# tgale96/sputnik

Hardware: AMD Instinct MI355X
Metric: effective TFLOP/s (nnz-FLOPs) DSD block=128 M=K=N=4096 @ 1/2/4/8 GPU vs density (higher is better)
Workload: dtype f16

## Files before the change

### sputnik_amd/csrc/dsd4w.hip

```cpp
#include <hip/hip_runtime.h>
#include <stdint.h>

#include <cstdlib>

#include "api_internal.h"
#include "block_gemm.h"
#include "dsd4w.h"
#include "dsd4w_asm.inc"

namespace sputnik_amd {
namespace {

constexpr int kRankScratch = 24576;
constexpr uint32_t kOob = 0x80000000u;

struct Pick {
  int row_a, row_b, e_a, n_a, e_b, n_b, target;
  int uniform;
};

__device__ Pick rank_wave(const GemmParams &p, char *lds, int wave, int lane,
                          int ra, int rb, int o0_pre, bool pre) {
  const int R = p.num_rows;
  const int o0 = pre ? o0_pre : lane <= R ? p.s_offsets[lane] : 0;
  const int o1 = __shfl_down(o0, 1, 64);
  const int nr = lane < R ? o1 - o0 : -1;
  int *keys = reinterpret_cast<int *>(lds + kRankScratch + wave * 256);
  int *nbr = reinterpret_cast<int *>(lds + kRankScratch + 2048 + wave * 256);
  const bool live = lane < R;
  const int key = live ? (nr << 6) | (63 - lane) : -1;
  keys[lane] = key;
  int4 k4[16];
#pragma unroll
  for (int j = 0; j < 16; ++j) k4[j] = *reinterpret_cast<const int4 *>(keys + 4 * j);
  int rank = 0;
#pragma unroll
  for (int j = 0; j < 16; ++j)
    rank += (k4[j].x > key) + (k4[j].y > key) + (k4[j].z > key) + (k4[j].w > key);
  const unsigned long long ba = __ballot(live && rank == ra);
  const unsigned long long bb = __ballot(live && rank == rb);
  Pick out;
  out.row_a = __builtin_ctzll(ba);
  out.row_b = __builtin_ctzll(bb);
  out.e_a = __builtin_amdgcn_readlane(o0, out.row_a);
  out.n_a = __builtin_amdgcn_readlane(nr, out.row_a);
  out.e_b = __builtin_amdgcn_readlane(o0, out.row_b);
  out.n_b = __builtin_amdgcn_readlane(nr, out.row_b);
  if (live) nbr[rank] = nr;
  int v = 0;
  if (lane < (R + 1) / 2) {
    const int j = R - 1 - lane;
    v = lane == j ? nbr[lane] : (nbr[lane] + nbr[j] + 1) / 2;
  }
  int vmax = 0;
#pragma unroll
  for (int bit = 15; bit >= 0; --bit) {
    const int cand = vmax | (1 << bit);
    if (__ballot(v >= cand) != 0) vmax = cand;
  }
  out.target = vmax;
  return out;
}

__device__ Pick rank_block(const GemmParams &p, char *lds, int tid, int ra, int rb) {
  const int R = p.num_rows;
  int *offs = reinterpret_cast<int *>(lds + kRankScratch);
  int *n_by_rank = offs + R + 1;
  int *scratch = reinterpret_cast<int *>(lds + kRankScratch + 4096);
  for (int r = tid; r <= R; r += 256) offs[r] = p.s_offsets[r];
  if (tid == 0) {
    scratch[2] = 0;
    scratch[3] = 1;
  }
  __syncthreads();
  const int n0 = offs[1] - offs[0];
  for (int r = tid; r < R; r += 256) {
    const int nr = offs[r + 1] - offs[r];
    if (nr != n0) scratch[3] = 0;
    int rank = 0;
    for (int r2 = 0; r2 < R; ++r2) {
      const int n2 = offs[r2 + 1] - offs[r2];
      rank += (n2 > nr) | ((n2 == nr) & (r2 < r));
    }
    n_by_rank[rank] = nr;
    if (rank == ra) scratch[0] = r;
    if (rank == rb) scratch[1] = r;
  }
  __syncthreads();
  for (int i = tid; i < (R + 1) / 2; i += 256) {
    const int j = R - 1 - i;
    const int v = i == j ? n_by_rank[i] : (n_by_rank[i] + n_by_rank[j] + 1) / 2;
    atomicMax(&scratch[2], v);
  }
  __syncthreads();
  Pick out;
  out.row_a = __builtin_amdgcn_readfirstlane(scratch[0]);
  out.row_b = __builtin_amdgcn_readfirstlane(scratch[1]);
  out.target = __builtin_amdgcn_readfirstlane(scratch[2]);
  out.uniform = __builtin_amdgcn_readfirstlane(scratch[3]);
  out.e_a = __builtin_amdgcn_readfirstlane(offs[out.row_a]);
  out.n_a = __builtin_amdgcn_readfirstlane(offs[out.row_a + 1]) - out.e_a;
  out.e_b = __builtin_amdgcn_readfirstlane(offs[out.row_b]);
  out.n_b = __builtin_amdgcn_readfirstlane(offs[out.row_b + 1]) - out.e_b;
  __syncthreads();
  return out;
}

__device__ __forceinline__ unsigned long long exp_stamp(int dep) {
#if (SPUTNIK_EXP & 512) != 0
  unsigned long long t;
  asm volatile("s_memrealtime %0\n s_waitcnt lgkmcnt(0)"
               : "=s"(t) : "s"(__builtin_amdgcn_readfirstlane(dep)));
  return t;
#else
  (void)dep;
  return 0;
#endif
}

template <bool kBf16, int kEpi, bool kDds, bool kSdd = false, bool kNt = false,
          bool kTt = false, bool kTn = false>
__global__ void __launch_bounds__(256, 1) dsd4w_kernel(const GemmParams p) {
  constexpr bool kWaveEpi = kEpi != 0;
  constexpr bool kDs = kEpi == 3 || kEpi == 4 || kEpi == 5 || kEpi == 6 || kEpi == 7;
  constexpr bool kBar2 = kEpi == 4;
  constexpr bool kKs = kEpi == 6;
  constexpr bool kTp = kEpi == 7;
  static_assert(!kTp || (!kSdd && !kDds && !kNt && !kTt && !kTn), "tall pipeline: DSD NN");
  static_assert(!kDds || kEpi == 1 || kEpi == 3, "DDS: per-wave epilogue only");
  static_assert(!kSdd || ((kEpi == 3 || (kEpi == 4 && !kTt) || (kEpi == 1 && kTn) ||
                           (kKs && !kNt && !kTt && !kTn)) && !kDds),
                "SDD: double slots (TN: per-step images), per-wave epilogue");
  static_assert(!kKs || kSdd, "K-split: SDD NN only");
  constexpr bool kARowsT = (kTt || kTn) && kSdd;
  constexpr bool kDdsTt = kDds && kTt;
  [[maybe_unused]] const unsigned long long t_entry = __builtin_amdgcn_s_memrealtime();
  __shared__ __attribute__((aligned(1024))) char lds[163840];
  const int tid = threadIdx.x;
  const int lane = tid & 63;
  const int wave = __builtin_amdgcn_readfirstlane(tid >> 6);
  const uint32_t lbase =
      (uint32_t)(uintptr_t)((__attribute__((address_space(3))) char *)lds);

  constexpr int kIdxPreload = 1024;
  const int nb_all = p.s_blocks;
  [[maybe_unused]] const unsigned long long t_karg = exp_stamp(nb_all);
  const bool idx_pre = nb_all <= kIdxPreload &&
                       (reinterpret_cast<uintptr_t>(p.s_indices) & 15) == 0;
  typedef unsigned v4u_t __attribute__((ext_vector_type(4)));
  v4u_t idx_lo = {0u, 0u, 0u, 0u}, idx_hi = {0u, 0u, 0u, 0u};
  if (idx_pre) {
    const __amdgpu_buffer_rsrc_t ri = __builtin_amdgcn_make_buffer_rsrc(
        const_cast<short *>(p.s_indices), 0, (nb_all * 2 + 3) & ~3, 0x00020000);
    idx_lo = __builtin_bit_cast(v4u_t, __builtin_amdgcn_raw_buffer_load_b128(
                                            ri, lane * 32, 0, 0));
    idx_hi = __builtin_bit_cast(v4u_t, __builtin_amdgcn_raw_buffer_load_b128(
                                            ri, lane * 32 + 16, 0, 0));
  }
#ifndef SPUTNIK_OFF_EARLY
#define SPUTNIK_OFF_EARLY 1
#endif
  const bool off_early = SPUTNIK_OFF_EARLY && !kSdd && !kTp && p.num_rows < 64;
  int off_pre = 0;
  if (off_early && lane <= p.num_rows) off_pre = p.s_offsets[lane];
  auto kblock_of = [&](int e) {
    if constexpr (kSdd) return e;
    if (!idx_pre || e >= nb_all) return scalar_load_short(p.s_indices, e);
    const int l = e >> 4, d = (e & 15) >> 1;
    const unsigned w0 = __builtin_amdgcn_readlane(idx_lo.x, l);
    const unsigned w1 = __builtin_amdgcn_readlane(idx_lo.y, l);
    const unsigned w2 = __builtin_amdgcn_readlane(idx_lo.z, l);
    const unsigned w3 = __builtin_amdgcn_readlane(idx_lo.w, l);
    const unsigned w4 = __builtin_amdgcn_readlane(idx_hi.x, l);
    const unsigned w5 = __builtin_amdgcn_readlane(idx_hi.y, l);
    const unsigned w6 = __builtin_amdgcn_readlane(idx_hi.z, l);
    const unsigned w7 = __builtin_amdgcn_readlane(idx_hi.w, l);
    const unsigned w = d == 0 ? w0 : d == 1 ? w1 : d == 2 ? w2 : d == 3 ? w3
                     : d == 4 ? w4 : d == 5 ? w5 : d == 6 ? w6 : w7;
    return (int)((e & 1) ? (w >> 16) : (w & 0xffff));
  };

  int srow, j0;
  int b1, n1, b2 = 0, n2 = 0;
  bool producer = false, collect = false;
  int pair_id = 0;
  [[maybe_unused]] unsigned long long t_rank = 0;
  unsigned epoch = p.pair_epoch;
  if (p.pair != 0 && p.pair_sync != nullptr)
    epoch = ((unsigned)scalar_load_int(reinterpret_cast<const int *>(p.pair_sync), 0) &
             0x7fffffffu) + 1u;
  int grp_b0 = 0, grp_count = 0, grp_c = 0;
  bool split_idle = false;
  int kss = 1, kch = 0, kofs = 0;
  unsigned tp_ent = 0, tp_tile = 0, tp_ent2 = 0, tp_tile2 = 0, tp_zero = 0xffffffffu;
  int tp_first = 0, tp_second = 0, tp_nzero = 0;
  if constexpr (kSdd) {
    int tile = xcd_tile(blockIdx.x, gridDim.x);
    const int R = !kKs && p.sdd_tail != 0
                      ? sdd_tail_rows<256>(p, reinterpret_cast<int *>(lds + kRankScratch), tid)
                      : p.num_rows;
    const bool band = p.sdd_order >= 1;
    const int per = band ? ((R + 255) / 256 + 7) & ~7 : (R + 255) / 256;
    const int r0 = min(R, tid * per), r1 = min(R, r0 + per);
    int local = 0, gmin = 0x7fffffff, gmax = 0;
    for (int r = r0; r < r1; ++r) {
      const int gr = (p.c_offsets[r + 1] - p.c_offsets[r] + 3) / 4;
      local += gr;
      gmin = min(gmin, gr);
      gmax = max(gmax, gr);
    }
    int incl = local;
#pragma unroll
    for (int d = 1; d < 64; d <<= 1) {
      const int v = __shfl_up(incl, d, 64);
      if (lane >= d) incl += v;
    }
#pragma unroll
    for (int d = 1; d < 64; d <<= 1) {
      gmin = min(gmin, __shfl_xor(gmin, d, 64));
      gmax = max(gmax, __shfl_xor(gmax, d, 64));
    }
    int *wsum = reinterpret_cast<int *>(lds + kRankScratch);
    if (lane == 63) {
      wsum[wave] = incl;
      wsum[4 + wave] = gmin;
      wsum[8 + wave] = gmax;
    }
    __syncthreads();
    int before = 0, total = 0;
    for (int w2 = 0; w2 < 4; ++w2) {
      const int v = wsum[w2];
      before += w2 < wave ? v : 0;
      total += v;
      gmin = min(gmin, wsum[4 + w2]);
      gmax = max(gmax, wsum[8 + w2]);
    }
    if constexpr (kKs) {
      const int nk = p.k_limit / 128;
      for (int s = 8; s >= 2 && kss == 1; s >>= 1)
        if (s <= p.sdd_ksplit && total * s <= (int)gridDim.x && nk >= 2 * s) kss = s;
      kch = tile / max(total, 1);
      tile -= kch * total;
      if (kch >= kss) tile = total;
    } else {
      tile = (int)blockIdx.x < total ? xcd_tile(blockIdx.x, total) : total;
    }
    int start = before + incl - local;
    const bool uniform = gmin == gmax;
    if (!uniform && band && total >= 8 * R) {
      for (int rb0 = r0; rb0 < r1; rb0 += 8) {
        int g8[8], bt = 0;
#pragma unroll
        for (int i = 0; i < 8; ++i) {
          g8[i] = rb0 + i < r1 ? (p.c_offsets[rb0 + i + 1] - p.c_offsets[rb0 + i] + 3) / 4 : 0;
          bt += g8[i];
        }
        if (tile >= start && tile < start + bt) {
          int o = tile - start, lo = 0;
          for (int it = 0; it < 8; ++it) {
            int cnt = 0, m = 0x7fffffff;
#pragma unroll
            for (int i = 0; i < 8; ++i)
              if (g8[i] > lo) {
                ++cnt;
                m = min(m, g8[i]);
              }
            if (o < cnt * (m - lo)) {
              const int k = o % cnt;
              int row = rb0, c = 0;
#pragma unroll
              for (int i = 0; i < 8; ++i)
                if (g8[i] > lo) {
                  if (c == k) row = rb0 + i;
                  ++c;
                }
              wsum[12] = row;
              wsum[13] = lo + o / cnt;
              break;
            }
            o -= cnt * (m - lo);
            lo = m;
          }
        }
        start += bt;
      }
    } else if (!uniform) {
      for (int r = r0; r < r1; ++r) {
        const int gr = (p.c_offsets[r + 1] - p.c_offsets[r] + 3) / 4;
        if (tile >= start && tile < start + gr) {
          wsum[12] = r;
          wsum[13] = tile - start;
        }
        start += gr;
      }
    }
    __syncthreads();
    j0 = 0;
    b1 = 0;
    n1 = p.k_limit / 128;
    srow = 0;
    if (tile >= total) {
      if (!kKs || p.pair == 0 || p.pair_sync == nullptr) return;
      split_idle = true;
    } else {
      int gi;
      const int gpr = total / max(R, 1);
      const int rb = p.sdd_order == 2 ? 4 : p.sdd_order == 3 ? 16 : p.sdd_order == 4 ? 32 : 8;
      const int gb = 32 / rb;
      if (uniform && p.sdd_order >= 1 && R % rb == 0 && gpr % gb == 0) {
        const int sup = tile >> 5, w = tile & 31;
        const int ngs = gpr / gb;
        srow = (sup / ngs) * rb + (w % rb);
        gi = p.sdd_spread ? (w / rb) * ngs + (sup % ngs) : (sup % ngs) * gb + (w / rb);
      } else if (uniform) {
        srow = tile % R;
        gi = tile / R;
      } else {
        srow = __builtin_amdgcn_readfirstlane(wsum[12]);
        gi = __builtin_amdgcn_readfirstlane(wsum[13]);
      }
      grp_b0 = __builtin_amdgcn_readfirstlane(p.c_offsets[srow] + gi * 4);
      grp_count = __builtin_amdgcn_readfirstlane(min(4, p.c_offsets[srow + 1] - grp_b0));
      grp_c = scalar_load_short(p.c_indices, grp_b0 + min(wave, grp_count - 1));
      if constexpr (kKs) {
        const int c0 = kch * n1 / kss, c1 = (kch + 1) * n1 / kss;
        kofs = c0;
        n1 = c1 - c0;
        pair_id = tile * kss;
      } else if (p.sdd_krot != 0 && n1 > 1) {
        const int key = p.sdd_krot == 1 ? srow : p.sdd_krot == 2 ? gi
                        : p.sdd_krot == 3 ? tile : srow >> 3;
        const int rot = (int)(((unsigned)key * 17u) % (unsigned)n1);
        b1 = rot;
        b2 = 0;
        n2 = rot;
        n1 -= rot;
      }
    }
    __syncthreads();
  } else if constexpr (kTp) {
    const int kFlushW = p.tall_flush_w;
    const int R = p.num_rows, NB = nb_all, P = p.num_jtiles;
    const int G = gridDim.x;
    const int w = xcd_tile(blockIdx.x, G);
    int *loff = reinterpret_cast<int *>(lds);
    int *wsc = reinterpret_cast<int *>(lds + kRankScratch + 131072);
    for (int r = tid; r <= R; r += 256) loff[r] = p.s_offsets[r];
    __syncthreads();
    const int per = (R + 255) / 256;
    const int r0 = min(R, tid * per), r1 = min(R, r0 + per);
    int local = 0;
    for (int r = r0; r < r1; ++r) local += loff[r + 1] == loff[r] ? 1 : 0;
    int incl = local;
#pragma unroll
    for (int d = 1; d < 64; d <<= 1) {
      const int v = __shfl_up(incl, d, 64);
      if (lane >= d) incl += v;
    }
    if (lane == 63) wsc[wave] = incl;
    __syncthreads();
    int before = 0, E = 0;
    for (int w2 = 0; w2 < 4; ++w2) {
      before += w2 < wave ? wsc[w2] : 0;
      E += wsc[w2];
    }
    const int NE = R - E;
    const long long W = 4LL * NB + (long long)kFlushW * NE;
    const long long TW = (long long)P * W;
    const int rot = xcd_rotation();
    auto share = [&](int ww) -> long long {
      long long acc = 0;
      int base = 0;
      for (int x = 0; x < 8; ++x) {
        const int nx = G / 8 + (x < G % 8 ? 1 : 0);
        const long long sx = fast_xcd(x, rot) ? p.tall_odd_share : 100;
        if (ww <= base + nx) return acc + (long long)(ww - base) * sx;
        acc += (long long)nx * sx;
        base += nx;
      }
      return acc;
    };
    const long long stot = share(G), sw0 = share(w), sw1 = share(w + 1);
    const long long lo0 = TW * sw0 / stot, lo1 = TW * sw1 / stot;
    const long long q0 = lo0 / max(W, 1LL), q1 = lo1 / max(W, 1LL);
    const long long rem0 = lo0 - q0 * W, rem1 = lo1 - q1 * W;
    long long m0 = (long long)NB, m1 = (long long)NB, k0 = 0x7fffffffffffLL, k1 = k0;
    {
      int e = before + incl - local;
      for (int r = r0; r < r1; ++r) {
        if (loff[r + 1] == loff[r]) {
          ++e;
          continue;
        }
        const long long key = 4LL * loff[r] + (long long)kFlushW * (r - e);
        if (key >= rem0 && key < k0) { k0 = key; m0 = loff[r]; }
        if (key >= rem1 && key < k1) { k1 = key; m1 = loff[r]; }
      }
    }
#pragma unroll
    for (int d = 1; d < 64; d <<= 1) {
      const long long ok0 = __shfl_xor(k0, d, 64), om0 = __shfl_xor(m0, d, 64);
      const long long ok1 = __shfl_xor(k1, d, 64), om1 = __shfl_xor(m1, d, 64);
      if (ok0 < k0) { k0 = ok0; m0 = om0; }
      if (ok1 < k1) { k1 = ok1; m1 = om1; }
    }
    long long *wk = reinterpret_cast<long long *>(wsc + 8);
    if (lane == 0) {
      wk[4 * wave] = k0;
      wk[4 * wave + 1] = m0;
      wk[4 * wave + 2] = k1;
      wk[4 * wave + 3] = m1;
    }
    __syncthreads();
    for (int w2 = 0; w2 < 4; ++w2) {
      if (wk[4 * w2] < k0) { k0 = wk[4 * w2]; m0 = wk[4 * w2 + 1]; }
      if (wk[4 * w2 + 2] < k1) { k1 = wk[4 * w2 + 2]; m1 = wk[4 * w2 + 3]; }
    }
    const long long T = (long long)P * NB;
    const long long b0 = min(T, q0 * NB + m0);
    const long long b1g = w + 1 == G ? T : min(T, q1 * NB + m1);
    const int nblk = (int)min(128LL, max(0LL, b1g - b0));
    auto describe = [&](int x, unsigned &ent, unsigned &til) {
      ent = 0;
      til = 0;
      if (x >= nblk) return;
      const long long g = b0 + x;
      const int q = (int)(g / NB), e = (int)(g - (long long)q * NB);
      int lo = 0, hi = R;
      while (hi - lo > 1) {
        const int mid = (lo + hi) >> 1;
        if (loff[mid] <= e) lo = mid; else hi = mid;
      }
      const bool last = e == loff[lo + 1] - 1;
      ent = (unsigned)e | ((unsigned)q << 24);
      til = (unsigned)lo | ((unsigned)q << 16) | (last ? 0x80000000u : 0u);
    };
    describe(lane, tp_ent, tp_tile);
    describe(64 + lane, tp_ent2, tp_tile2);
    {
      const long long Z = (long long)P * E;
      const int zlo = (int)(Z * sw0 / stot), zhi = (int)(Z * sw1 / stot);
      int *zl = wsc + 48;
      int e = before + incl - local;
      for (int r = r0; r < r1; ++r) {
        if (loff[r + 1] != loff[r]) continue;
        for (int q = 0; q < P; ++q) {
          const long long rank = (long long)q * E + e;
          if (rank >= zlo && rank < zhi) zl[rank - zlo] = r | (q << 16);
        }
        ++e;
      }
      __syncthreads();
      tp_nzero = min(64, zhi - zlo);
      tp_zero = lane < tp_nzero ? (unsigned)zl[lane] : 0xffffffffu;
    }
    __syncthreads();
    j0 = 0;
    srow = 0;
    b1 = 0;
    n1 = nblk;
    tp_first = (int)(__builtin_amdgcn_readlane(tp_ent, 0) & 0xffffffu);
    tp_second = (int)(__builtin_amdgcn_readlane(tp_ent, nblk > 1 ? 1 : 0) & 0xffffffu);
    split_idle = nblk == 0;
  } else if (p.pair != 0 && p.pair_split == 2) {
    const int nt = p.num_tiles;
    const int gch = (int)blockIdx.x >= nt ? 1 : 0;
    const int t = xcd_tile((int)blockIdx.x - gch * nt, nt);
    srow = t % p.num_rows;
    j0 = (t / p.num_rows) * 512;
    const int e_r = scalar_load_int(p.s_offsets, srow);
    const int n_r = scalar_load_int(p.s_offsets, srow + 1) - e_r;
    const int c0 = gch * n_r / 2, c1 = (gch + 1) * n_r / 2;
    b1 = e_r + c0;
    n1 = c1 - c0;
    pair_id = t;
    if (gch == 0) {
      producer = n1 > 0;
      split_idle = n1 == 0;
    } else {
      collect = n_r / 2 > 0;
    }
  } else if (p.pair != 0) {
    const int R = p.num_rows;
    const int half = R >> 1;
    const int n_light = p.num_jtiles * half;
    const int n_solo = p.num_jtiles * (R & 1);
    const int bid = blockIdx.x;
    int role, panel, pi;
    const bool xcd2 = p.pair_xcd2 != 0 && p.num_jtiles == 8 && n_solo == 0 &&
                      (half & 1) == 0;
    const int rot = xcd2 ? xcd_rotation() : 0;
    auto place = [&](int b) {
      if (xcd2) {
        const int x = b & 7, k = b >> 3;
        panel = 2 * (x >> 1) + (k & 1);
        pi = p.pair_xcd2 == 2 ? 2 * (k >> 1) + (x & 1)
           : (fast_xcd(x, rot) ^ (p.pair_xcd2 == 3 ? 1 : 0)) * (half >> 1) + (k >> 1);
      } else {
        const int t = xcd_tile(b, n_light);
        panel = t / half;
        pi = t % half;
      }
    };
    if (bid < n_light) {
      role = 0;
      place(bid);
    } else if (bid < n_light + n_solo) {
      role = 1;
      panel = bid - n_light;
      pi = half;
    } else {
      role = 2;
      place(bid - n_light - n_solo);
    }
    const Pick rp = R < 64 ? rank_wave(p, lds, wave, lane, pi, R - 1 - pi, off_pre, off_early)
                           : rank_block(p, lds, tid, pi, R - 1 - pi);
    t_rank = exp_stamp(rp.target + rp.e_a + rp.e_b);
    const int min_handoff = p.min_handoff > 0 ? p.min_handoff : SPUTNIK_MIN_HANDOFF;
    int hb = role == 1 ? 0 : rp.n_a - rp.target;
    if (hb < min_handoff) hb = 0;
    pair_id = panel * half + pi;
    j0 = panel * 512;
    if (role == 0) {
      srow = rp.row_b;
      b1 = rp.e_a;
      n1 = hb;
      b2 = rp.e_b;
      n2 = rp.n_b;
      producer = hb > 0;
    } else {
      srow = rp.row_a;
      b1 = rp.e_a + hb;
      n1 = rp.n_a - hb;
      collect = hb > 0;
    }
  } else {
    const int tile = xcd_tile(blockIdx.x, gridDim.x);
    const int panel = tile / p.num_rows;
    const int target = tile % p.num_rows;
    j0 = panel * 512;
    if (p.num_rows < 64) {
      const Pick rp = rank_wave(p, lds, wave, lane, target, target, off_pre, off_early);
      srow = rp.row_a;
      b1 = rp.e_a;
      n1 = rp.n_a;
    } else if (p.num_rows <= kLptRows) {
      const Pick rp = rank_block(p, lds, tid, target, target);
      srow = rp.row_a;
      b1 = rp.e_a;
      n1 = rp.n_a;
      const int R = p.num_rows;
      if (p.xcd_rows != 0 && rp.uniform != 0 && (R & 7) == 0 &&
          (int)gridDim.x == p.num_tiles) {
        const int rx = R >> 3, x = (int)blockIdx.x & 7, tx = (int)blockIdx.x >> 3;
        srow = x * rx + tx % rx;
        j0 = (tx / rx) * 512;
        const int *offs = reinterpret_cast<const int *>(lds + kRankScratch);
        b1 = __builtin_amdgcn_readfirstlane(offs[srow]);
      }
    } else {
      srow = target;
      b1 = scalar_load_int(p.s_offsets, srow);
      n1 = scalar_load_int(p.s_offsets, srow + 1) - b1;
    }
  }
  srow = __builtin_amdgcn_readfirstlane(srow);
  j0 = __builtin_amdgcn_readfirstlane(j0);
  const int ntot = n1 + n2;

  typedef unsigned v4u __attribute__((ext_vector_type(4)));
  if (split_idle) {
  } else if (ntot == 0 && kDds) {
    const v4u z = {0u, 0u, 0u, 0u};
    for (int id = tid; id < 512 * 16; id += 256) {
      const int r = id >> 4, cc = id & 15;
      if (j0 + r >= p.j_limit) continue;
      __builtin_nontemporal_store(
          z, reinterpret_cast<v4u *>(p.c_data + (long long)(j0 + r) * p.c_ld +
                                     (long long)srow * 256 + cc * 16));
    }
  } else if (ntot == 0) {
    const v4u z = {0u, 0u, 0u, 0u};
    for (int id = tid; id < 128 * 64; id += 256) {
      const int r = id >> 6, cc = id & 63;
      const int jc = j0 + cc * 8;
      if (jc >= p.j_limit) continue;
      __builtin_nontemporal_store(
          z, reinterpret_cast<v4u *>(p.c_data + ((long long)srow * 128 + r) * p.c_ld +
                                     (long long)jc * 2));
    }
  } else {
    const int b2m = b2 - n1;
    const int xlast = ntot - 1;
    auto entry = [&](int x) { return x + (x < n1 ? b1 : b2m); };
    const int kb0 = kblock_of(kTp ? tp_first : entry(0));
    const int kb1 = kblock_of(kTp ? tp_second : entry(xlast < 1 ? xlast : 1));
    constexpr bool kColOrder =
        !kDdsTt && ((kDds && !kNt) || ((kTn || kTt) && !kSdd));
    const int bo0 = kColOrder ? scalar_load_int(p.s_block_offsets, entry(0)) : 0;
    const int bo1 =
        kColOrder ? scalar_load_int(p.s_block_offsets, entry(xlast < 1 ? xlast : 1)) : 0;
    [[maybe_unused]] const unsigned long long t_kb = exp_stamp(kb0 + kb1);

    uint32_t vs, vs1 = 0;
    if constexpr (!kDdsTt && ((kDds && !kNt) || kTt || kTn)) {
      const int k = 8 * wave + (lane >> 4);
      const int pc = lane & 15;
      const int c = (((pc >> 1) ^ tr_key(k)) << 1) | (pc & 1);
      vs = (uint32_t)(k * (kARowsT ? p.s_ld : 256) + c * 16);
    } else if constexpr (kDs) {
      const long long srs = kSdd ? p.s_ld : 256;
      auto off = [&](int x) {
        const int r = 32 * wave + 8 * x + (lane >> 3);
        return (uint32_t)(r * srs + (((lane & 7) ^ ((r >> 1) & 7)) << 4));
      };
      vs = off(0);
      vs1 = off(1);
    } else {
      const int srow_l = 32 * wave + (lane >> 2);
      vs = (uint32_t)(srow_l * 256 + (((lane & 3) ^ ((srow_l >> 1) & 3)) << 4));
    }
    uint32_t vd[2];
#pragma unroll
    for (int x = 0; x < 2; ++x) {
      if constexpr (!kDdsTt && ((kDds && kDs) || kNt || kTt)) {
        const int r = 8 * x + (lane >> 3);
        vd[x] = j0 + 128 * wave < p.j_limit
                    ? (uint32_t)(r * p.d_ld + (((lane & 7) ^ ((r >> 1) & 7)) << 4))
                    : kOob;
      } else if constexpr (kDds && !kTn && !kDdsTt) {
        const int r = lane >> 2;
        vd[x] = j0 + 128 * wave < p.j_limit
                    ? (uint32_t)(r * p.d_ld + (((lane & 3) ^ ((r >> 1) & 3)) << 4))
                    : kOob;
      } else {
        const int k = (lane >> 4) + 8 * x;
        const int pc = lane & 15;
        const int c = (((pc >> 1) ^ tr_key(k)) << 1) | (pc & 1);
        const int col = (kSdd ? grp_c * 128 : j0 + 128 * wave) + c * 8;
        vd[x] = col < p.j_limit ? (uint32_t)((lane >> 4) * p.d_ld + c * 16) : kOob;
      }
    }
    const uint32_t own = lbase + 32768u + 32768u * wave;
    const int r16 = lane & 15, g = lane >> 4;
    const uint32_t vrs =
        (kDds ? own : lbase) +
        (kDs ? (uint32_t)(r16 * 128 + ((g ^ ((r16 >> 1) & 7)) << 4))
             : (uint32_t)(r16 * 64 + ((g ^ ((r16 >> 1) & 3)) << 4)));
    const uint32_t vrs1 = vrs ^ 64u;
    const int q = (lane >> 2) & 3, pp = lane & 3;
    const int kr = 8 * g + q;
    uint32_t vrd[8];
#pragma unroll
    for (int n = 0; n < 8; ++n)
      vrd[n] = (kDds || kTt ? lbase : own) +
               (uint32_t)(kr * 256 + pp * 8 + ((n ^ tr_key(kr)) << 5));
    uint32_t vrt[8];
#pragma unroll
    for (int m = 0; m < 8; ++m)
      vrt[m] = (kDds ? own : lbase) +
               (uint32_t)(kr * 256 + pp * 8 + ((m ^ tr_key(kr)) << 5));
    const uint32_t vrk0 = (kDds ? lbase : own) +
                          (uint32_t)(r16 * 128 + ((g ^ ((r16 >> 1) & 7)) << 4));
    const uint32_t vrk1 = vrk0 ^ 64u;
    const uint32_t vw0 = lbase + (uint32_t)(r16 * 1040 + (128 * wave + 4 * g) * 2);
    const uint32_t vw1 = vw0 + 64 * 1040;
    const uint32_t wreg = lbase + 32768u + 32768u * wave;
    uint32_t vws[8], vrb[4];
#pragma unroll
    for (int n = 0; n < 8; ++n)
      vws[n] = wreg + (uint32_t)(r16 * 256 + (((2 * n + (g >> 1)) ^ r16) << 4) + 8 * (g & 1));
#pragma unroll
    for (int qq = 0; qq < 4; ++qq) {
      const int rr = 4 * qq + g;
      vrb[qq] = wreg + (uint32_t)(rr * 256 + ((r16 ^ rr) << 4));
    }
    const bool cvalid = kSdd   ? wave < grp_count
                        : kDds ? j0 + 128 * wave < p.j_limit
                               : j0 + 128 * wave + r16 * 8 < p.j_limit;
    const long long cld = kSdd ? 256 : p.c_ld;
    const uint32_t vco = cvalid ? (uint32_t)(g * cld + r16 * 16) : kOob;
    const uint32_t vpl = (uint32_t)(wave * 65536 + lane * 16);
    const uint32_t vcl = (uint32_t)((lane & 15) * p.c_ld + (lane >> 4) * 8);

    auto U = [](uint32_t x) { return (uint32_t)__builtin_amdgcn_readfirstlane((int)x); };
    auto U64 = [&](uint64_t x) {
      return (uint64_t)U((uint32_t)x) | ((uint64_t)U((uint32_t)(x >> 32)) << 32);
    };
    const uint64_t sd = U64((uint64_t)(
        p.s_data + (kARowsT ? (long long)srow * 256
                    : kSdd  ? (long long)srow * 128 * p.s_ld + (long long)kofs * 256 : 0)));
    const uint64_t dt = U64((uint64_t)(
        p.d_data + (kDdsTt ? (long long)(j0 + 128 * wave) * 2
                    : (kNt || kTt) && !kSdd ? (long long)(j0 + 128 * wave) * p.d_ld
                    : kNt || kTt ? (long long)grp_c * 128 * p.d_ld
                    : kSdd ? (long long)grp_c * 256 + (long long)kofs * 128 * p.d_ld
                           : (long long)(j0 + 128 * wave) * (kDds && !kTn ? p.d_ld : 2))));
    const uint64_t ix = U64((uint64_t)p.s_indices);
    const uint64_t pd =
        U64((uint64_t)(p.pair_partials + (long long)pair_id * 128 * 512));
    const uint64_t flag_p =
        U64(kKs ? (uint64_t)(p.ks_flags + pair_id)
            : p.pair != 0 ? (uint64_t)(p.pair_flags + pair_id) : 0);
    const uint64_t err_p = U64((uint64_t)p.pair_error);
    constexpr bool kKcD = !kDdsTt && ((kDds && !kTn) || kNt || kTt);
    const uint32_t k128 = U((uint32_t)(kKcD ? 256 : 128 * p.d_ld));
    const uint32_t k32 = U((uint32_t)(kKcD ? 64 : 32 * p.d_ld));
    const uint32_t k4 = U((uint32_t)(kKcD ? 16 * p.d_ld : 4 * p.d_ld));
    const uint32_t ms =
        U(lbase + ((kDs && (((!kDds || kNt) && !kTt) || kDdsTt)) ? 4096u : 2048u) * wave);
    const uint32_t sk32 = U((uint32_t)(kARowsT ? 32 * p.s_ld : 0));
    const uint32_t sk128 = U((uint32_t)(kARowsT ? 128 * p.s_ld : 0));
    const uint32_t md = U(lbase + 32768u + 32768u * wave);
    const uint32_t flushrem = U(producer ? (uint32_t)n2 : 0xffffffffu);
    const uint32_t pubat = U(producer && n2 > 0 ? (uint32_t)n2 + 1u : 0u);
    const uint32_t publast = U(producer && n2 == 0 ? 1u : 0u);
    const bool clb = collect && ntot >= 3;
    const uint32_t clbf = U(clb ? 2u : 0xffffffffu), clbc = U(clb ? 1u : 0xffffffffu);
    const bool split_first = p.pair != 0 && p.pair_split == 2 && producer;
    const uint32_t flags =
        U((collect ? 1u : 0u) | (!collect && !(producer && n2 == 0) ? 2u : 0u) |
          (p.pair_fault ? 4u : 0u) | (wave == 3 ? 8u : 0u) | (wave == 0 ? 16u : 0u) |
          (split_first ? 32u : 0u) | (kKs && wave >= grp_count ? 64u : 0u));
    const uint64_t cd = U64(
        kSdd ? (uint64_t)(p.c_data + (long long)(grp_b0 + wave) * 32768)
        : kDds ? (uint64_t)(p.c_data + (long long)(j0 + 128 * wave) * p.c_ld +
                          (long long)srow * 256)
             : (uint64_t)(p.c_data + (long long)srow * 128 * p.c_ld +
                          (long long)(j0 + 128 * wave) * 2));
    const uint64_t bo = U64((uint64_t)p.s_block_offsets);
    const uint32_t c4 = U((uint32_t)(4 * cld));
    const uint32_t s16 = U((uint32_t)(kARowsT ? 4 * p.s_ld : kSdd ? 16 * p.s_ld : 0));
    const uint32_t ub1 = U(b1), un1 = U(n1), ub2m = U(b2m), uxlast = U(xlast),
                   untot = U(ntot), ukb0 = U(kb0), ukb1 = U(kb1), uep = U(epoch),
                   ubo0 = U(bo0), ubo1 = U(bo1), ukss = U(kss), ukch = U(kch);
    const uint32_t crow = U((uint32_t)(128 * p.c_ld));
    const uint32_t unz = U((uint32_t)tp_nzero);

#define DSD4W_INPUTS                                                           \
    [sdlo] "s"((uint32_t)sd), [sdhi] "s"((uint32_t)(sd >> 32)),               \
    [dtlo] "s"((uint32_t)dt), [dthi] "s"((uint32_t)(dt >> 32)),               \
    [k128] "s"(k128), [k32] "s"(k32), [k4] "s"(k4),                            \
    [ixlo] "s"((uint32_t)ix), [ixhi] "s"((uint32_t)(ix >> 32)),               \
    [b1] "s"(ub1), [n1] "s"(un1), [b2m] "s"(ub2m), [xlast] "s"(uxlast),        \
    [ntot] "s"(untot), [kb0] "s"(ukb0), [kb1] "s"(ukb1),                       \
    [flushrem] "s"(flushrem),                                                  \
    [pdlo] "s"((uint32_t)pd), [pdhi] "s"((uint32_t)(pd >> 32)),               \
    [flag] "s"(flag_p), [epoch] "s"(uep), [flags] "s"(flags),                  \
    [err] "s"(err_p), [ms] "s"(ms),                                            \
    [md] "s"(md), [vs] "v"(vs), [vd0] "v"(vd[0]), [vd1] "v"(vd[1]),           \
    [vrs] "v"(vrs), [vrd0] "v"(vrd[0]), [vrd1] "v"(vrd[1]),                   \
    [vs1] "v"(vs1), [vrs1] "v"(vrs1), [s16] "s"(s16),                          \
    [vrk0] "v"(vrk0), [vrk1] "v"(vrk1), [sk32] "s"(sk32), [sk128] "s"(sk128),  \
    [vrt0] "v"(vrt[0]), [vrt1] "v"(vrt[1]), [vrt2] "v"(vrt[2]), [vrt3] "v"(vrt[3]), \
    [vrt4] "v"(vrt[4]), [vrt5] "v"(vrt[5]), [vrt6] "v"(vrt[6]), [vrt7] "v"(vrt[7]), \
    [vrd2] "v"(vrd[2]), [vrd3] "v"(vrd[3]), [vrd4] "v"(vrd[4]),               \
    [vrd5] "v"(vrd[5]), [vrd6] "v"(vrd[6]), [vrd7] "v"(vrd[7]),               \
    [vpl] "v"(vpl), [bolo] "s"((uint32_t)bo), [bohi] "s"((uint32_t)(bo >> 32)),  \
    [bo0] "s"(ubo0), [bo1] "s"(ubo1), [pubat] "s"(pubat), [clbf] "s"(clbf),  \
    [clbc] "s"(clbc), [publast] "s"(publast), [kss] "s"(ukss), [kch] "s"(ukch), \
    [vent] "v"(tp_ent), [vtile] "v"(tp_tile), [vent2] "v"(tp_ent2),         \
    [vtile2] "v"(tp_tile2), [vcl] "v"(vcl), [crow] "s"(crow),                \
    [vzero] "v"(tp_zero), [nzero] "s"(unz)
#define DSD4W_OPERANDS : DSD4W_INPUTS
#define DSD4W_OPERANDS_G DSD4W_OPERANDS, [vw0] "v"(vw0), [vw1] "v"(vw1)
#define DSD4W_INPUTS_W                                                         \
  DSD4W_INPUTS, [cdlo] "s"((uint32_t)cd), [cdhi] "s"((uint32_t)(cd >> 32)),  \
      [c4] "s"(c4), [vws0] "v"(vws[0]), [vws1] "v"(vws[1]), [vws2] "v"(vws[2]), \
      [vws3] "v"(vws[3]), [vws4] "v"(vws[4]), [vws5] "v"(vws[5]),               \
      [vws6] "v"(vws[6]), [vws7] "v"(vws[7]), [vrb0] "v"(vrb[0]),               \
      [vrb1] "v"(vrb[1]), [vrb2] "v"(vrb[2]), [vrb3] "v"(vrb[3]), [vco] "v"(vco)
#define DSD4W_OPERANDS_W : DSD4W_INPUTS_W
#define DSD4W_RECORD(ROLE, EXTRA)                                              \
  if (p.debug != nullptr && wave == 0 && lane < 16) {                          \
    unsigned long long v = 0;                                                  \
    v = lane == 0 ? t_entry : v;                                               \
    v = lane == 1 ? t_asm : v;                                                 \
    v = lane == 2 ? r0 : v;                                                    \
    v = lane == 3 ? r1 : v;                                                    \
    v = lane == 4 ? r2 : v;                                                    \
    v = lane == 5 ? (unsigned long long)ntot : v;                              \
    v = lane == 6 ? (ROLE) : v;                                                \
    v = lane == 7 ? (unsigned long long)srow : v;                              \
    v = lane == 8 ? (unsigned long long)n1 : v;                                \
    v = lane == 9 ? r3 : v;                                                    \
    v = lane == 10 ? r4 : v;                                                   \
    v = lane == 11 ? t_karg : v;                                               \
    v = lane == 12 ? t_rank : v;                                               \
    v = lane == 13 ? t_kb : v;                                                 \
    v = lane == 14 ? (EXTRA) : v;                                              \
    p.debug[blockIdx.x * 16 + lane] = v;                                       \
  }
    if constexpr (kDdsTt) {
      if constexpr (kBf16)
        asm volatile(DSD4W_ASM_BF16_W2_DDS_TT : DSD4W_OPERANDS_W : DSD4W_CLOBBERS);
      else
        asm volatile(DSD4W_ASM_F16_W2_DDS_TT : DSD4W_OPERANDS_W : DSD4W_CLOBBERS);
    } else if constexpr (kTt && !kSdd) {
      if constexpr (kBf16)
        asm volatile(DSD4W_ASM_BF16_W2_TT : DSD4W_OPERANDS_W : DSD4W_CLOBBERS);
      else
        asm volatile(DSD4W_ASM_F16_W2_TT : DSD4W_OPERANDS_W : DSD4W_CLOBBERS);
    } else if constexpr (kTn && kSdd) {
      if constexpr (kBf16)
        asm volatile(DSD4W_ASM_BF16_W_SDD_TN : DSD4W_OPERANDS_W : DSD4W_CLOBBERS);
      else
        asm volatile(DSD4W_ASM_F16_W_SDD_TN : DSD4W_OPERANDS_W : DSD4W_CLOBBERS);
    } else if constexpr (kTn && kDds) {
      if constexpr (kBf16)
        asm volatile(DSD4W_ASM_BF16_W_DDS_TN : DSD4W_OPERANDS_W : DSD4W_CLOBBERS);
      else
        asm volatile(DSD4W_ASM_F16_W_DDS_TN : DSD4W_OPERANDS_W : DSD4W_CLOBBERS);
    } else if constexpr (kTn) {
      if constexpr (kBf16)
        asm volatile(DSD4W_ASM_BF16_W_TN : DSD4W_OPERANDS_W : DSD4W_CLOBBERS);
      else
        asm volatile(DSD4W_ASM_F16_W_TN : DSD4W_OPERANDS_W : DSD4W_CLOBBERS);
    } else if constexpr (kTt) {
      if constexpr (kBf16)
        asm volatile(DSD4W_ASM_BF16_W2_SDD_TT : DSD4W_OPERANDS_W : DSD4W_CLOBBERS);
      else
        asm volatile(DSD4W_ASM_F16_W2_SDD_TT : DSD4W_OPERANDS_W : DSD4W_CLOBBERS);
    } else if constexpr (kNt && kDds) {
      if constexpr (kBf16)
        asm volatile(DSD4W_ASM_BF16_W2_DDS_NT : DSD4W_OPERANDS_W : DSD4W_CLOBBERS);
      else
        asm volatile(DSD4W_ASM_F16_W2_DDS_NT : DSD4W_OPERANDS_W : DSD4W_CLOBBERS);
    } else if constexpr (kNt && !kSdd) {
      if constexpr (kBf16)
        asm volatile(DSD4W_ASM_BF16_W2_NT : DSD4W_OPERANDS_W : DSD4W_CLOBBERS);
      else
        asm volatile(DSD4W_ASM_F16_W2_NT : DSD4W_OPERANDS_W : DSD4W_CLOBBERS);
    } else if constexpr (kNt && kBar2) {
      if constexpr (kBf16)
        asm volatile(DSD4W_ASM_BF16_W3_SDD_NT : DSD4W_OPERANDS_W : DSD4W_CLOBBERS);
      else
        asm volatile(DSD4W_ASM_F16_W3_SDD_NT : DSD4W_OPERANDS_W : DSD4W_CLOBBERS);
    } else if constexpr (kNt) {
      if constexpr (kBf16)
        asm volatile(DSD4W_ASM_BF16_W2_SDD_NT : DSD4W_OPERANDS_W : DSD4W_CLOBBERS);
      else
        asm volatile(DSD4W_ASM_F16_W2_SDD_NT : DSD4W_OPERANDS_W : DSD4W_CLOBBERS);
    } else if constexpr (kTp && (SPUTNIK_EXP & 512) != 0) {
      const unsigned long long t_asm = __builtin_amdgcn_s_memrealtime();
      unsigned long long r0 = 0, r1 = 0, r2 = 0, r3 = 0, r4 = 0;
      if constexpr ((SPUTNIK_EXP & 1024) != 0)
        asm volatile(DSD4W_ASM_F16_W2_TP_NS : [r0] "=&s"(r0), [r1] "=&s"(r1),
                     [r2] "=&s"(r2), [r3] "=&s"(r3), [r4] "=&s"(r4)
                     : DSD4W_INPUTS_W : DSD4W_CLOBBERS);
      else if constexpr (kBf16)
        asm volatile(DSD4W_ASM_BF16_W2_TP_T : [r0] "=&s"(r0), [r1] "=&s"(r1),
                     [r2] "=&s"(r2), [r3] "=&s"(r3), [r4] "=&s"(r4)
                     : DSD4W_INPUTS_W : DSD4W_CLOBBERS);
      else
        asm volatile(DSD4W_ASM_F16_W2_TP_T : [r0] "=&s"(r0), [r1] "=&s"(r1),
                     [r2] "=&s"(r2), [r3] "=&s"(r3), [r4] "=&s"(r4)
                     : DSD4W_INPUTS_W : DSD4W_CLOBBERS);
      const unsigned long long ntl = (unsigned long long)(
          __popcll(__ballot((tp_tile >> 31) != 0)) + __popcll(__ballot((tp_tile2 >> 31) != 0)));
      DSD4W_RECORD((unsigned long long)tp_nzero, ntl);
    } else if constexpr (kTp) {
      if constexpr (kBf16)
        asm volatile(DSD4W_ASM_BF16_W2_TP : DSD4W_OPERANDS_W : DSD4W_CLOBBERS);
      else
        asm volatile(DSD4W_ASM_F16_W2_TP : DSD4W_OPERANDS_W : DSD4W_CLOBBERS);
    } else if constexpr (kKs && (SPUTNIK_EXP & 512) != 0) {
      const unsigned long long t_asm = __builtin_amdgcn_s_memrealtime();
      unsigned long long r0 = 0, r1 = 0, r2 = 0, r3 = 0, r4 = 0;
      if constexpr (kBf16)
        asm volatile(DSD4W_ASM_BF16_W2_SDD_KS_T : [r0] "=&s"(r0), [r1] "=&s"(r1),
                     [r2] "=&s"(r2), [r3] "=&s"(r3), [r4] "=&s"(r4)
                     : DSD4W_INPUTS_W : DSD4W_CLOBBERS);
      else
        asm volatile(DSD4W_ASM_F16_W2_SDD_KS_T : [r0] "=&s"(r0), [r1] "=&s"(r1),
                     [r2] "=&s"(r2), [r3] "=&s"(r3), [r4] "=&s"(r4)
                     : DSD4W_INPUTS_W : DSD4W_CLOBBERS);
      DSD4W_RECORD((unsigned long long)kch, (unsigned long long)kss);
    } else if constexpr (kKs) {
      if constexpr (kBf16)
        asm volatile(DSD4W_ASM_BF16_W2_SDD_KS : DSD4W_OPERANDS_W : DSD4W_CLOBBERS);
      else
        asm volatile(DSD4W_ASM_F16_W2_SDD_KS : DSD4W_OPERANDS_W : DSD4W_CLOBBERS);
    } else if constexpr (kSdd && kBar2) {
      if constexpr (kBf16)
        asm volatile(DSD4W_ASM_BF16_W3_SDD : DSD4W_OPERANDS_W : DSD4W_CLOBBERS);
      else
        asm volatile(DSD4W_ASM_F16_W3_SDD : DSD4W_OPERANDS_W : DSD4W_CLOBBERS);
    } else if constexpr (kSdd) {
      if constexpr (kBf16)
        asm volatile(DSD4W_ASM_BF16_W2_SDD : DSD4W_OPERANDS_W : DSD4W_CLOBBERS);
      else
        asm volatile(DSD4W_ASM_F16_W2_SDD : DSD4W_OPERANDS_W : DSD4W_CLOBBERS);
    } else if constexpr (kDds && kDs && (SPUTNIK_EXP & 512) != 0) {
      const unsigned long long t_asm = __builtin_amdgcn_s_memrealtime();
      unsigned long long r0 = 0, r1 = 0, r2 = 0, r3 = 0, r4 = 0;
      if constexpr (kBf16)
        asm volatile(DSD4W_ASM_BF16_W2_DDS_T : [r0] "=&s"(r0), [r1] "=&s"(r1),
                     [r2] "=&s"(r2), [r3] "=&s"(r3), [r4] "=&s"(r4)
                     : DSD4W_INPUTS_W : DSD4W_CLOBBERS);
      else
        asm volatile(DSD4W_ASM_F16_W2_DDS_T : [r0] "=&s"(r0), [r1] "=&s"(r1),
                     [r2] "=&s"(r2), [r3] "=&s"(r3), [r4] "=&s"(r4)
                     : DSD4W_INPUTS_W : DSD4W_CLOBBERS);
      DSD4W_RECORD((unsigned long long)((collect ? 2 : 0) | (producer ? 1 : 0)), 0ull);
    } else if constexpr (kDds && kDs) {
      if constexpr (kBf16)
        asm volatile(DSD4W_ASM_BF16_W2_DDS : DSD4W_OPERANDS_W : DSD4W_CLOBBERS);
      else
        asm volatile(DSD4W_ASM_F16_W2_DDS : DSD4W_OPERANDS_W : DSD4W_CLOBBERS);
    } else if constexpr (kDds) {
      if constexpr (kBf16)
        asm volatile(DSD4W_ASM_BF16_W_DDS : DSD4W_OPERANDS_W : DSD4W_CLOBBERS);
      else
        asm volatile(DSD4W_ASM_F16_W_DDS : DSD4W_OPERANDS_W : DSD4W_CLOBBERS);
    } else if constexpr ((SPUTNIK_EXP & 512) != 0 &&
                         (kEpi == 1 || kEpi == 3 || kEpi == 5)) {
      const unsigned long long t_asm = __builtin_amdgcn_s_memrealtime();
      unsigned long long r0 = 0, r1 = 0, r2 = 0, r3 = 0, r4 = 0;
#define DSD4W_STAMPED(NAME)                                                    \
  asm volatile(NAME : [r0] "=&s"(r0), [r1] "=&s"(r1), [r2] "=&s"(r2),          \
               [r3] "=&s"(r3), [r4] "=&s"(r4)                                  \
               : DSD4W_INPUTS_W : DSD4W_CLOBBERS)
      if constexpr (kEpi == 5) {
        if constexpr (kBf16) DSD4W_STAMPED(DSD4W_ASM_BF16_W4_T);
        else DSD4W_STAMPED(DSD4W_ASM_F16_W4_T);
      } else if constexpr (kEpi == 3) {
        if constexpr (kBf16) DSD4W_STAMPED(DSD4W_ASM_BF16_W2_T);
        else DSD4W_STAMPED(DSD4W_ASM_F16_W2_T);
      } else {
        if constexpr (kBf16) DSD4W_STAMPED(DSD4W_ASM_BF16_W_T);
        else DSD4W_STAMPED(DSD4W_ASM_F16_W_T);
      }
#undef DSD4W_STAMPED
      DSD4W_RECORD((unsigned long long)((collect ? 2 : 0) | (producer ? 1 : 0)), 0ull);
    } else if constexpr (kEpi == 5) {
      if constexpr (kBf16)
        asm volatile(DSD4W_ASM_BF16_W4 : DSD4W_OPERANDS_W : DSD4W_CLOBBERS);
      else
        asm volatile(DSD4W_ASM_F16_W4 : DSD4W_OPERANDS_W : DSD4W_CLOBBERS);
    } else if constexpr (kBar2) {
      if constexpr (kBf16)
        asm volatile(DSD4W_ASM_BF16_W3 : DSD4W_OPERANDS_W : DSD4W_CLOBBERS);
      else
        asm volatile(DSD4W_ASM_F16_W3 : DSD4W_OPERANDS_W : DSD4W_CLOBBERS);
    } else if constexpr (kDs) {
      if constexpr (kBf16)
        asm volatile(DSD4W_ASM_BF16_W2 : DSD4W_OPERANDS_W : DSD4W_CLOBBERS);
      else
        asm volatile(DSD4W_ASM_F16_W2 : DSD4W_OPERANDS_W : DSD4W_CLOBBERS);
    } else if constexpr (kEpi == 2) {
      if constexpr (kBf16)
        asm volatile(DSD4W_ASM_BF16_WL : DSD4W_OPERANDS_W : DSD4W_CLOBBERS);
      else
        asm volatile(DSD4W_ASM_F16_WL : DSD4W_OPERANDS_W : DSD4W_CLOBBERS);
    } else if constexpr (kWaveEpi) {
      if constexpr (kBf16)
        asm volatile(DSD4W_ASM_BF16_W : DSD4W_OPERANDS_W : DSD4W_CLOBBERS);
      else
        asm volatile(DSD4W_ASM_F16_W : DSD4W_OPERANDS_W : DSD4W_CLOBBERS);
    } else {
      if constexpr (kBf16)
        asm volatile(DSD4W_ASM_BF16 : DSD4W_OPERANDS_G : DSD4W_CLOBBERS);
      else
        asm volatile(DSD4W_ASM_F16 : DSD4W_OPERANDS_G : DSD4W_CLOBBERS);
      __syncthreads();
      for (int id = tid; id < 128 * 64; id += 256) {
        const int r = id >> 6, cc = id & 63;
        const int jc = j0 + cc * 8;
        if (jc >= p.j_limit) continue;
        const v4u v = *reinterpret_cast<const v4u *>(lds + r * 1040 + cc * 16);
        __builtin_nontemporal_store(
            v, reinterpret_cast<v4u *>(p.c_data + ((long long)srow * 128 + r) * p.c_ld +
                                       (long long)jc * 2));
      }
    }
#undef DSD4W_RECORD
#undef DSD4W_OPERANDS_W
#undef DSD4W_INPUTS_W
#undef DSD4W_OPERANDS_G
#undef DSD4W_OPERANDS
#undef DSD4W_INPUTS
  }
  if constexpr (kTp) {
    typedef unsigned v4z __attribute__((ext_vector_type(4)));
    const v4z z = {0u, 0u, 0u, 0u};
    int jz = 0;
    if (!split_idle) {
// ... 205 lines not shown
```

Measured before the change: 1184.

## Hoist per-lane LDS address setup ahead of scheduling and use DPP reductions

New measurement: 1190 (median of 6 runs). Within noise of the previous version (+0.5%).

```diff
diff --git a/sputnik_amd/csrc/dsd4w.hip b/sputnik_amd/csrc/dsd4w.hip
--- a/sputnik_amd/csrc/dsd4w.hip
+++ b/sputnik_amd/csrc/dsd4w.hip
@@ -26,7 +26,6 @@
   const int o1 = __shfl_down(o0, 1, 64);
   const int nr = lane < R ? o1 - o0 : -1;
   int *keys = reinterpret_cast<int *>(lds + kRankScratch + wave * 256);
-  int *nbr = reinterpret_cast<int *>(lds + kRankScratch + 2048 + wave * 256);
   const bool live = lane < R;
   const int key = live ? (nr << 6) | (63 - lane) : -1;
   keys[lane] = key;
@@ -46,19 +45,17 @@
   out.n_a = __builtin_amdgcn_readlane(nr, out.row_a);
   out.e_b = __builtin_amdgcn_readlane(o0, out.row_b);
   out.n_b = __builtin_amdgcn_readlane(nr, out.row_b);
-  if (live) nbr[rank] = nr;
+  const int by_rank = __builtin_amdgcn_ds_permute(rank << 2, live ? nr : 0);
+  const int j = R - 1 - lane;
+  const int partner = __builtin_amdgcn_ds_bpermute(j << 2, by_rank);
   int v = 0;
-  if (lane < (R + 1) / 2) {
-    const int j = R - 1 - lane;
-    v = lane == j ? nbr[lane] : (nbr[lane] + nbr[j] + 1) / 2;
-  }
-  int vmax = 0;
-#pragma unroll
-  for (int bit = 15; bit >= 0; --bit) {
-    const int cand = vmax | (1 << bit);
-    if (__ballot(v >= cand) != 0) vmax = cand;
-  }
-  out.target = vmax;
+  if (lane < (R + 1) / 2) v = lane == j ? by_rank : (by_rank + partner + 1) / 2;
+  v = max(v, __builtin_amdgcn_update_dpp(0, v, 0xB1, 0xf, 0xf, true));
+  v = max(v, __builtin_amdgcn_update_dpp(0, v, 0x4E, 0xf, 0xf, true));
+  v = max(v, __builtin_amdgcn_update_dpp(0, v, 0x141, 0xf, 0xf, true));
+  v = max(v, __builtin_amdgcn_update_dpp(0, v, 0x140, 0xf, 0xf, true));
+  out.target = max(max(__builtin_amdgcn_readlane(v, 0), __builtin_amdgcn_readlane(v, 16)),
+                   max(__builtin_amdgcn_readlane(v, 32), __builtin_amdgcn_readlane(v, 48)));
   return out;
 }
 
@@ -167,18 +164,98 @@
     if constexpr (kSdd) return e;
     if (!idx_pre || e >= nb_all) return scalar_load_short(p.s_indices, e);
     const int l = e >> 4, d = (e & 15) >> 1;
-    const unsigned w0 = __builtin_amdgcn_readlane(idx_lo.x, l);
-    const unsigned w1 = __builtin_amdgcn_readlane(idx_lo.y, l);
-    const unsigned w2 = __builtin_amdgcn_readlane(idx_lo.z, l);
-    const unsigned w3 = __builtin_amdgcn_readlane(idx_lo.w, l);
-    const unsigned w4 = __builtin_amdgcn_readlane(idx_hi.x, l);
-    const unsigned w5 = __builtin_amdgcn_readlane(idx_hi.y, l);
-    const unsigned w6 = __builtin_amdgcn_readlane(idx_hi.z, l);
-    const unsigned w7 = __builtin_amdgcn_readlane(idx_hi.w, l);
-    const unsigned w = d == 0 ? w0 : d == 1 ? w1 : d == 2 ? w2 : d == 3 ? w3
-                     : d == 4 ? w4 : d == 5 ? w5 : d == 6 ? w6 : w7;
+    const v4u_t h = (d & 4) ? idx_hi : idx_lo;
+    const unsigned h0 = (d & 2) ? h.z : h.x, h1 = (d & 2) ? h.w : h.y;
+    const unsigned w = __builtin_amdgcn_readlane((d & 1) ? h1 : h0, l);
     return (int)((e & 1) ? (w >> 16) : (w & 0xffff));
   };
+
+  uint32_t vs, vs1 = 0;
+  if constexpr (!kDdsTt && ((kDds && !kNt) || kTt || kTn)) {
+    const int k = 8 * wave + (lane >> 4);
+    const int pc = lane & 15;
+    const int c = (((pc >> 1) ^ tr_key(k)) << 1) | (pc & 1);
+    vs = (uint32_t)(k * (kARowsT ? p.s_ld : 256) + c * 16);
+  } else if constexpr (kDs) {
+    const long long srs = kSdd ? p.s_ld : 256;
+    auto off = [&](int x) {
+      const int r = 32 * wave + 8 * x + (lane >> 3);
+      return (uint32_t)(r * srs + (((lane & 7) ^ ((r >> 1) & 7)) << 4));
+    };
+    vs = off(0);
+    vs1 = off(1);
+  } else {
+    const int srow_l = 32 * wave + (lane >> 2);
+    vs = (uint32_t)(srow_l * 256 + (((lane & 3) ^ ((srow_l >> 1) & 3)) << 4));
+  }
+  uint32_t vd_off[2], vd_col[2];
+#pragma unroll
+  for (int x = 0; x < 2; ++x) {
+    if constexpr (!kDdsTt && ((kDds && kDs) || kNt || kTt)) {
+      const int r = 8 * x + (lane >> 3);
+      vd_off[x] = (uint32_t)(r * p.d_ld + (((lane & 7) ^ ((r >> 1) & 7)) << 4));
+      vd_col[x] = (uint32_t)(128 * wave);
+    } else if constexpr (kDds && !kTn && !kDdsTt) {
+      const int r = lane >> 2;
+      vd_off[x] = (uint32_t)(r * p.d_ld + (((lane & 3) ^ ((r >> 1) & 3)) << 4));
+      vd_col[x] = (uint32_t)(128 * wave);
+    } else {
+      const int k = (lane >> 4) + 8 * x;
+      const int pc = lane & 15;
+      const int c = (((pc >> 1) ^ tr_key(k)) << 1) | (pc & 1);
+      vd_off[x] = (uint32_t)((lane >> 4) * p.d_ld + c * 16);
+      vd_col[x] = (uint32_t)((kSdd ? 0 : 128 * wave) + c * 8);
+    }
+  }
+  const uint32_t own = lbase + 32768u + 32768u * wave;
+  const int r16 = lane & 15, g = lane >> 4;
+  uint32_t vrs =
+      (kDds ? own : lbase) +
+      (kDs ? (uint32_t)(r16 * 128 + ((g ^ ((r16 >> 1) & 7)) << 4))
+           : (uint32_t)(r16 * 64 + ((g ^ ((r16 >> 1) & 3)) << 4)));
+  uint32_t vrs1 = vrs ^ 64u;
+  const int q = (lane >> 2) & 3, pp = lane & 3;
+  const int kr = 8 * g + q;
+  uint32_t vrd[8];
+#pragma unroll
+  for (int n = 0; n < 8; ++n)
+    vrd[n] = (kDds || kTt ? lbase : own) +
+             (uint32_t)(kr * 256 + pp * 8 + ((n ^ tr_key(kr)) << 5));
+  uint32_t vrt[8];
+#pragma unroll
+  for (int m = 0; m < 8; ++m)
+    vrt[m] = (kDds ? own : lbase) +
+             (uint32_t)(kr * 256 + pp * 8 + ((m ^ tr_key(kr)) << 5));
+  uint32_t vrk0 = (kDds ? lbase : own) +
+                        (uint32_t)(r16 * 128 + ((g ^ ((r16 >> 1) & 7)) << 4));
+  uint32_t vrk1 = vrk0 ^ 64u;
+  uint32_t vw0 = lbase + (uint32_t)(r16 * 1040 + (128 * wave + 4 * g) * 2);
+  uint32_t vw1 = vw0 + 64 * 1040;
+  const uint32_t wreg = lbase + 32768u + 32768u * wave;
+  uint32_t vws[8], vrb[4];
+#pragma unroll
+  for (int n = 0; n < 8; ++n)
+    vws[n] = wreg + (uint32_t)(r16 * 256 + (((2 * n + (g >> 1)) ^ r16) << 4) + 8 * (g & 1));
+#pragma unroll
+  for (int qq = 0; qq < 4; ++qq) {
+    const int rr = 4 * qq + g;
+    vrb[qq] = wreg + (uint32_t)(rr * 256 + ((r16 ^ rr) << 4));
+  }
+  uint32_t vpl = (uint32_t)(wave * 65536 + lane * 16);
+  uint32_t vcl = (uint32_t)((lane & 15) * p.c_ld + (lane >> 4) * 8);
+  if constexpr (!kSdd && !kTp) {
+#define DSD4W_PIN(x) asm volatile("" : "+v"(x))
+    DSD4W_PIN(vs); DSD4W_PIN(vs1); DSD4W_PIN(vrs); DSD4W_PIN(vrs1);
+    DSD4W_PIN(vrk0); DSD4W_PIN(vrk1); DSD4W_PIN(vw0); DSD4W_PIN(vw1);
+    DSD4W_PIN(vpl); DSD4W_PIN(vcl);
+#pragma unroll
+    for (int x = 0; x < 2; ++x) { DSD4W_PIN(vd_off[x]); DSD4W_PIN(vd_col[x]); }
+#pragma unroll
+    for (int n = 0; n < 8; ++n) { DSD4W_PIN(vrd[n]); DSD4W_PIN(vrt[n]); DSD4W_PIN(vws[n]); }
+#pragma unroll
+    for (int n = 0; n < 4; ++n) DSD4W_PIN(vrb[n]);
+#undef DSD4W_PIN
+  }
 
   int srow, j0;
   int b1, n1, b2 = 0, n2 = 0;
@@ -602,87 +679,18 @@
         kColOrder ? scalar_load_int(p.s_block_offsets, entry(xlast < 1 ? xlast : 1)) : 0;
     [[maybe_unused]] const unsigned long long t_kb = exp_stamp(kb0 + kb1);
 
-    uint32_t vs, vs1 = 0;
-    if constexpr (!kDdsTt && ((kDds && !kNt) || kTt || kTn)) {
-      const int k = 8 * wave + (lane >> 4);
-      const int pc = lane & 15;
-      const int c = (((pc >> 1) ^ tr_key(k)) << 1) | (pc & 1);
-      vs = (uint32_t)(k * (kARowsT ? p.s_ld : 256) + c * 16);
-    } else if constexpr (kDs) {
-      const long long srs = kSdd ? p.s_ld : 256;
-      auto off = [&](int x) {
-        const int r = 32 * wave + 8 * x + (lane >> 3);
-        return (uint32_t)(r * srs + (((lane & 7) ^ ((r >> 1) & 7)) << 4));
-      };
-      vs = off(0);
-      vs1 = off(1);
-    } else {
-      const int srow_l = 32 * wave + (lane >> 2);
-      vs = (uint32_t)(srow_l * 256 + (((lane & 3) ^ ((srow_l >> 1) & 3)) << 4));
-    }
+    constexpr bool kGrpCol = kSdd && !(!kDdsTt && ((kDds && kDs) || kNt || kTt)) &&
+                             !(kDds && !kTn && !kDdsTt);
+    const int dbase = kGrpCol ? grp_c * 128 : j0;
     uint32_t vd[2];
 #pragma unroll
-    for (int x = 0; x < 2; ++x) {
-      if constexpr (!kDdsTt && ((kDds && kDs) || kNt || kTt)) {
-        const int r = 8 * x + (lane >> 3);
-        vd[x] = j0 + 128 * wave < p.j_limit
-                    ? (uint32_t)(r * p.d_ld + (((lane & 7) ^ ((r >> 1) & 7)) << 4))
-                    : kOob;
-      } else if constexpr (kDds && !kTn && !kDdsTt) {
-        const int r = lane >> 2;
-        vd[x] = j0 + 128 * wave < p.j_limit
-                    ? (uint32_t)(r * p.d_ld + (((lane & 3) ^ ((r >> 1) & 3)) << 4))
-                    : kOob;
-      } else {
-        const int k = (lane >> 4) + 8 * x;
-        const int pc = lane & 15;
-        const int c = (((pc >> 1) ^ tr_key(k)) << 1) | (pc & 1);
-        const int col = (kSdd ? grp_c * 128 : j0 + 128 * wave) + c * 8;
-        vd[x] = col < p.j_limit ? (uint32_t)((lane >> 4) * p.d_ld + c * 16) : kOob;
-      }
-    }
-    const uint32_t own = lbase + 32768u + 32768u * wave;
-    const int r16 = lane & 15, g = lane >> 4;
-    const uint32_t vrs =
-        (kDds ? own : lbase) +
-        (kDs ? (uint32_t)(r16 * 128 + ((g ^ ((r16 >> 1) & 7)) << 4))
-             : (uint32_t)(r16 * 64 + ((g ^ ((r16 >> 1) & 3)) << 4)));
-    const uint32_t vrs1 = vrs ^ 64u;
-    const int q = (lane >> 2) & 3, pp = lane & 3;
-    const int kr = 8 * g + q;
-    uint32_t vrd[8];
-#pragma unroll
-    for (int n = 0; n < 8; ++n)
-      vrd[n] = (kDds || kTt ? lbase : own) +
-               (uint32_t)(kr * 256 + pp * 8 + ((n ^ tr_key(kr)) << 5));
-    uint32_t vrt[8];
-#pragma unroll
-    for (int m = 0; m < 8; ++m)
-      vrt[m] = (kDds ? own : lbase) +
-               (uint32_t)(kr * 256 + pp * 8 + ((m ^ tr_key(kr)) << 5));
-    const uint32_t vrk0 = (kDds ? lbase : own) +
-                          (uint32_t)(r16 * 128 + ((g ^ ((r16 >> 1) & 7)) << 4));
-    const uint32_t vrk1 = vrk0 ^ 64u;
-    const uint32_t vw0 = lbase + (uint32_t)(r16 * 1040 + (128 * wave + 4 * g) * 2);
-    const uint32_t vw1 = vw0 + 64 * 1040;
-    const uint32_t wreg = lbase + 32768u + 32768u * wave;
-    uint32_t vws[8], vrb[4];
-#pragma unroll
-    for (int n = 0; n < 8; ++n)
-      vws[n] = wreg + (uint32_t)(r16 * 256 + (((2 * n + (g >> 1)) ^ r16) << 4) + 8 * (g & 1));
-#pragma unroll
-    for (int qq = 0; qq < 4; ++qq) {
-      const int rr = 4 * qq + g;
-      vrb[qq] = wreg + (uint32_t)(rr * 256 + ((r16 ^ rr) << 4));
-    }
+    for (int x = 0; x < 2; ++x)
+      vd[x] = dbase + (int)vd_col[x] < p.j_limit ? vd_off[x] : kOob;
     const bool cvalid = kSdd   ? wave < grp_count
                         : kDds ? j0 + 128 * wave < p.j_limit
                                : j0 + 128 * wave + r16 * 8 < p.j_limit;
     const long long cld = kSdd ? 256 : p.c_ld;
     const uint32_t vco = cvalid ? (uint32_t)(g * cld + r16 * 16) : kOob;
-    const uint32_t vpl = (uint32_t)(wave * 65536 + lane * 16);
-    const uint32_t vcl = (uint32_t)((lane & 15) * p.c_ld + (lane >> 4) * 8);
-
     auto U = [](uint32_t x) { return (uint32_t)__builtin_amdgcn_readfirstlane((int)x); };
     auto U64 = [&](uint64_t x) {
       return (uint64_t)U((uint32_t)x) | ((uint64_t)U((uint32_t)(x >> 32)) << 32);
```
